# Alxaline/BraTS21

Hardware: AMD Instinct MI355X
Metric: train patches/sec (4x128^3, width-48) (higher is better)
Workload: dtype bf16; 1 GPU; equiunet width=48, batch=2/GPU of 4x128^3 synthetic patches, fwd + deep-supervision Dice + bwd + ranger (BASELINE.json configs[1]); global_batch=2, parallelism=dp1

## Files before the change

### brats21_amd/_lib.py

```python
import ctypes
import os
import re

_HERE = os.path.dirname(os.path.abspath(__file__))
LIB_PATH = os.environ.get("BRATS_HIP_LIB") or os.path.join(_HERE, "libbrats_hip.so")
HEADER_PATH = os.path.join(os.path.dirname(_HERE), "include", "brats_hip.h")

F32, BF16, F16, X3_BF16, X3_F16 = 0, 1, 2, 3, 4
ACT_NONE, ACT_RELU, ACT_LEAKY, ACT_ELU, ACT_SWISH, ACT_MISH = 0, 1, 2, 3, 4, 5
PACK_FWD, PACK_DGRAD = 0, 1


class BratsHipError(RuntimeError):
    pass


_C = {"p": ctypes.c_void_p, "i": ctypes.c_int, "f": ctypes.c_float, "d": ctypes.c_double, "z": ctypes.c_size_t}

def _parse_header():
    txt = open(HEADER_PATH).read()
    txt = re.sub(r"/\*.*?\*/", " ", txt, flags=re.S)
    sigs = {}
    for m in re.finditer(r"(const char\s*\*|size_t|int)\s+(brats_[a-z0-9_]+)\s*\(([^)]*)\)\s*;", txt):
        ret, name, args = m.group(1), m.group(2), m.group(3).strip()
        spec = ""
        if args and args != "void":
            for a in args.split(","):
                a = a.strip()
                if "*" in a or "brats_stream_t" in a:
                    spec += "p"
                elif a.startswith("size_t"):
                    spec += "z"
                elif a.startswith("double"):
                    spec += "d"
                elif a.startswith("float"):
                    spec += "f"
                elif a.startswith("int"):
                    spec += "i"
                else:
                    raise BratsHipError(f"cannot bind argument '{a}' of {name}")
        sigs[name] = ("s" if "char" in ret else ("z" if ret == "size_t" else "i"), spec)
    return sigs

# ... 51 lines not shown
```

### brats21_amd/csrc/dice.hip

```cpp
#include "common.hpp"

__global__ void dice_stats_kernel(const float* __restrict__ x, const float* __restrict__ t, float* __restrict__ part, int K,
                                  size_t voxels) {
  const int nk = blockIdx.y, k = nk % K;
  const float* xp = x + (size_t)nk * voxels;
  const float* tp = t + (size_t)nk * voxels;
  float s0 = 0.f, s1 = 0.f, s2 = 0.f;
  const size_t v4 = voxels / 4;
  for (size_t i = (size_t)blockIdx.x * blockDim.x + threadIdx.x; i < v4; i += (size_t)gridDim.x * blockDim.x) {
    const f32x4 xv = ((const f32x4*)xp)[i], tv = ((const f32x4*)tp)[i];
#pragma unroll
    for (int j = 0; j < 4; ++j) {
      const float p = 1.f / (1.f + __expf(-xv[j]));
      s0 += tv[j] * p;
      s1 += p * p;
      s2 += tv[j] * tv[j];
    }
  }
  if (blockIdx.x == 0) {
    for (size_t i = v4 * 4 + threadIdx.x; i < voxels; i += blockDim.x) {
      const float p = 1.f / (1.f + __expf(-xp[i]));
      s0 += tp[i] * p; s1 += p * p; s2 += tp[i] * tp[i];
    }
  }
// ... 68 lines not shown
  }
  if (blockIdx.x == 0) {
    for (size_t i = v4 * 4 + threadIdx.x; i < voxels; i += blockDim.x) {
      const float p = 1.f / (1.f + __expf(-xp[i]));
      dp[i] = (a * tp[i] + b2 * p) * p * (1.f - p);
    }
  }
}

constexpr int DICE_MAX_BLOCKS = 512;
extern "C" size_t brats_dice_ws_floats(int N, int K) { return (size_t)N * DICE_MAX_BLOCKS * K * 3; }

extern "C" int brats_dice_stats(const float* logits, const float* target, float* sums , float* ws, int N, int K,
                                size_t voxels, brats_stream_t s) {
  if (!logits || !target || !sums || !ws || N <= 0 || K <= 0) BRATS_FAIL(BRATS_E_ARG, "dice_stats: bad argument");
  hipStream_t st = (hipStream_t)s;
  size_t gx = (voxels / 4 + 255) / 256 / 4;
  gx = gx < 1 ? 1 : (gx > DICE_MAX_BLOCKS ? DICE_MAX_BLOCKS : gx);
  hipLaunchKernelGGL(dice_stats_kernel, dim3((unsigned)gx, N * K), dim3(256), 0, st, logits, target, ws, K, voxels);
  brats_ordered_sum(ws, sums, N * (int)gx, K * 3, st);
  BRATS_CHECK_LAUNCH();
  return 0;
}

extern "C" int brats_dice_grad(const float* logits, const float* target, const float* coef ,
                               float* dlogits, int N, int K, size_t voxels, brats_stream_t s) {
  if (!logits || !target || !coef || !dlogits) BRATS_FAIL(BRATS_E_ARG, "dice_grad: null pointer");
  size_t gx = (voxels / 4 + 255) / 256 / 4;
  gx = gx < 1 ? 1 : (gx > 2048 ? 2048 : gx);
  hipLaunchKernelGGL(dice_grad_kernel, dim3((unsigned)gx, N * K), dim3(256), 0, (hipStream_t)s, logits, target, coef, dlogits, K, voxels);
  BRATS_CHECK_LAUNCH();
  return 0;
}
```

### brats21_amd/engine.py

```python
import torch

from . import ops
from .evaluate import Evaluator
from .losses import DiceLoss, deep_supervision_loss, fused_deep_supervision_dice


class TrainStep:

    def __init__(self, model, optimizer, criterion=None, amp=True, buckets=None, fused_dice=True, jaccard=False,
                 max_grad_norm=None, amp_dtype=torch.bfloat16, scaler=None):
        self.model, self.optimizer, self.amp, self.buckets = model, optimizer, amp, buckets
        self.fused, self.jaccard, self.max_grad_norm = fused_dice and criterion is None, jaccard, max_grad_norm
        self.criterion = criterion if criterion is not None else DiceLoss(jaccard=jaccard)
        self.amp_dtype = amp_dtype
        self.scaler = scaler
        self._params = None
        if amp and amp_dtype == torch.float16 and scaler is None:
            self.scaler = torch.amp.GradScaler("cuda")

    def loss(self, outputs, target):
        if self.fused:
            return fused_deep_supervision_dice(outputs, target, jaccard=self.jaccard)
        return deep_supervision_loss(self.criterion, outputs, target)[0]

    def _zero_grad(self):
        params = self._params
        if params is None:
            params = self._params = list(self.model.parameters())
        for p in params:
            p.grad = None

    def __call__(self, image, target):
        self._zero_grad()
        with torch.autocast("cuda", dtype=self.amp_dtype, enabled=self.amp):
            outputs = self.model(image)
            loss = self.loss(outputs, target)
        if self.scaler is not None and self.amp:
            self.scaler.scale(loss).backward()
            if self.buckets is not None:
                self.buckets.finish()
            if self.max_grad_norm is not None:
                self.scaler.unscale_(self.optimizer)
                torch.nn.utils.clip_grad_norm_(self.model.parameters(), self.max_grad_norm)
            self.scaler.step(self.optimizer)
            self.scaler.update()
            return loss
        loss.backward()
        if self.buckets is not None:
            self.buckets.finish()
        if self.max_grad_norm is not None:
            torch.nn.utils.clip_grad_norm_(self.model.parameters(), self.max_grad_norm)
        self.optimizer.step()
        return loss


class GraphedTrainStep:

    def __init__(self, step, warmup=2, multi_rank_capture=None):
        if getattr(step, "scaler", None) is not None and step.amp:
            if not (getattr(step.optimizer, "_step_supports_amp_scaling", False) and getattr(step.optimizer, "capturable", False)) \
                    or step.max_grad_norm is not None:
                raise NotImplementedError("GraphedTrainStep: a TrainStep with a GradScaler (amp_dtype=torch.float16) captures only with "
                                          "an optimizer that implements the GradScaler protocol on the device "
                                          "(brats21_amd.optim.Ranger2020(capturable=True)) and without gradient clipping; otherwise use "
                                          "the eager TrainStep for fp16, or bf16 / model.precision='x3' for graph replay")
        if step.buckets is not None:
            import os
            import torch.distributed as dist
# ... 47 lines not shown
```

### brats21_amd/losses.py

```python
import torch
import torch.nn as nn


class DiceLoss(nn.Module):
    def __init__(self, jaccard=False, smooth_nr=1e-5, smooth_dr=1e-5):
        super().__init__()
        self.jaccard, self.smooth_nr, self.smooth_dr = jaccard, smooth_nr, smooth_dr

    def forward(self, logits, target):
        p = torch.sigmoid(logits.float())
        t = target.float()
        axes = (0, 2, 3, 4)
        inter = (t * p).sum(axes)
        denom = (t * t).sum(axes) + (p * p).sum(axes)
        if self.jaccard:
            denom = 2.0 * (denom - inter)
        return (1.0 - (2.0 * inter + self.smooth_nr) / (denom + self.smooth_dr)).mean()


def deep_supervision_loss(criterion, outputs, target):
    if isinstance(outputs, (tuple, list)):
        heads = [outputs[0]] + list(outputs[1])
        return torch.stack([criterion(h, target) for h in heads]).mean(), outputs[0]
    return criterion(outputs, target), outputs


class _FusedDiceFn(torch.autograd.Function):

    @staticmethod
    def forward(ctx, target, jaccard, eps, *heads):
        from . import _lib
        lib = _lib.lib()
        st = torch.cuda.current_stream().cuda_stream
        t = target.contiguous().float()
        n, k = t.shape[:2]
        vox = t[0, 0].numel()
        hs = [h.contiguous().float() for h in heads]
        sums = torch.empty((len(hs), k, 3), dtype=torch.float32, device=t.device)
        ws = torch.empty(lib.brats_dice_ws_floats(n, k), dtype=torch.float32, device=t.device)
        for i, h in enumerate(hs):
            _lib.check(lib.brats_dice_stats(h.data_ptr(), t.data_ptr(), sums[i].data_ptr(), ws.data_ptr(), n, k, vox, st), "dice_stats")
        inter, p2, t2 = sums[..., 0], sums[..., 1], sums[..., 2]
        hk = float(len(hs) * k)
        if jaccard:
            den = 2.0 * (t2 + p2 - inter)
            f = 1.0 - (2.0 * inter + eps) / (den + eps)
            dden = (2.0 * inter + eps) / (den + eps) ** 2
            coef = torch.stack([(-2.0 / (den + eps) - 2.0 * dden) / hk, 2.0 * dden / hk], -1)
        else:
            den = t2 + p2
            f = 1.0 - (2.0 * inter + eps) / (den + eps)
            coef = torch.stack([-2.0 / (den + eps) / hk, (2.0 * inter + eps) / (den + eps) ** 2 / hk], -1)
        ctx.save_for_backward(t, coef.contiguous(), *hs)
        return f.mean()

    @staticmethod
    def backward(ctx, g):
        from . import _lib
        lib = _lib.lib()
        st = torch.cuda.current_stream().cuda_stream
        t, coef, *hs = ctx.saved_tensors
        n, k = t.shape[:2]
        vox = t[0, 0].numel()
        coef = (coef * g).contiguous()
        outs = []
        for i, h in enumerate(hs):
            d = torch.empty_like(h)
            _lib.check(lib.brats_dice_grad(h.data_ptr(), t.data_ptr(), coef[i].data_ptr(), d.data_ptr(), n, k, vox, st), "dice_grad")
            outs.append(d)
        return (None, None, None) + tuple(outs)


def fused_deep_supervision_dice(outputs, target, jaccard=False, eps=1e-5):
    heads = [outputs[0]] + list(outputs[1]) if isinstance(outputs, (tuple, list)) else [outputs]
    return _FusedDiceFn.apply(target, jaccard, eps, *heads)
```

### brats21_amd/networks/equiunet.py

```python
import contextlib
import math

import os

import torch
import torch.nn as nn

from .. import ops
from .._lib import PACK_DGRAD, PACK_FWD, BratsHipError


class _ConvParams(nn.Module):

    def __init__(self, cin, cout, k, bias):
        super().__init__()
        self.weight = nn.Parameter(torch.empty(cout, cin, k, k, k))
        self.bias = nn.Parameter(torch.empty(cout)) if bias else None
        nn.init.kaiming_uniform_(self.weight, a=math.sqrt(5))
        if bias:
            bound = 1.0 / math.sqrt(cin * k * k * k)
            nn.init.uniform_(self.bias, -bound, bound)


class _NormParams(nn.Module):
# ... 415 lines not shown
        down1, p1 = cgr(m.encoder1.ConvBnRelu2, cgr(m.encoder1.ConvBnRelu1, x0, lazy=True), pool=True)
        down2, p2 = cgr(m.encoder2.ConvBnRelu2, cgr(m.encoder2.ConvBnRelu1, p1, lazy=True), pool=True)
        down3, p3 = cgr(m.encoder3.ConvBnRelu2, cgr(m.encoder3.ConvBnRelu1, p2, lazy=True), pool=True)
        down4 = cgr(m.encoder4.ConvBnRelu2, cgr(m.encoder4.ConvBnRelu1, p3, lazy=True))
        deep_heads = m.deep_supervision and not (m.skip_deep_heads_in_eval and not m.training)
        bottom = cgr(m.bottom.ConvBnRelu2, cgr(m.bottom.ConvBnRelu1, down4, lazy=True), lazy=not deep_heads)
        bottom_2 = cgr(m.bottom_2, down4, x2=bottom)
        up3 = cgr(m.decoder3.ConvBnRelu2, cgr(m.decoder3.ConvBnRelu1, down3, x2=up(bottom_2), lazy=True))
        up2 = cgr(m.decoder2.ConvBnRelu2, cgr(m.decoder2.ConvBnRelu1, down2, x2=up(up3), lazy=True))
        u1 = cgr(m.decoder1.ConvBnRelu1, down1, x2=up(up2), lazy=True)
        kact, slope_t = _unit_act(m.decoder1.ConvBnRelu2, act)
        nk = m.outconv.weight.shape[0]
        fuse_top = (m.fold_head_fwd and drop_state is None and not m.decoder1.ConvBnRelu2.batch_norm and slope_t is None and kact in ("relu", "leakyrelu") and nk <= 4
                    and (not will_bwd or (m.fold_head_bwd and ops.head_fold_ok(m.outconv.weight, kact, slope_t))))
        if fuse_top:
            y1, rec1 = _cgr_fwd(m.decoder1.ConvBnRelu2, u1, dtype, act, None, None, fp8, slots, no_act=True)
            tape.append(rec1)
            up1 = None
            outs = [ops.gn_head(y1, rec1[5], m.outconv.weight, m.outconv.bias, kact)]
        else:
            up1 = cgr(m.decoder1.ConvBnRelu2, u1)
            outs = [ops.head(up1, m.outconv.weight, m.outconv.bias, 1)]
        ctx.top_fused = fuse_top
        ctx.out_shape = tuple(outs[0].shape)
        heads = [(m.outconv, up1, 1)]
        if deep_heads:
            for hd, src, sc in ((m.deep_bottom[0], bottom, 8), (m.deep_bottom2[0], bottom_2, 8), (m.deep3[0], up3, 4),
                                (m.deep2[0], up2, 2)):
                outs.append(ops.head(src, hd.weight, hd.bias, sc))
                heads.append((hd, src, sc))
        ctx.model, ctx.dtype, ctx.tape, ctx.heads = m, dtype, tape, heads
        ctx.bufs = (down1, down2, down3, down4, bottom, bottom_2, up3, up2, up1)
        ctx.nparams = len(params)
        return tuple(outs)

    @staticmethod
    def _backward(ctx, *douts):
        m, dtype, tape = ctx.model, ctx.dtype, ctx.tape
        act, f = m.act, m.features
        names = {p: i for i, p in enumerate(m.parameters())}
        grads = {}
        down1, down2, down3, down4, bottom, bottom_2, up3, up2, up1 = ctx.bufs
        rec = {r[0]: r for r in tape}

        fp8 = m.conv_fp8 if ops.is16(dtype) else None
        slots = _AmaxSlots(32, douts[0].device) if (fp8 == "all" or ops.x3_mode() == ops.X3F) else None

        drop_state = ctx.drop_state

        def cbw(unit, dz, need_dx=True, head=None, pool=None, first=None):
            bst = rec[first] if (first is not None and m.fold_bwd_stats and drop_state is None) else None
            drop = (m.dropout_p, drop_state, m._unit_ids[unit]) if drop_state is not None else None
            return _cgr_bwd(rec[unit], dz, dtype, act, grads, names, need_dx, m._grad_sink, fp8, slots, m._grad_dest, head, pool, bst,
                            drop)

        def level_bwd(unit, down, d_pooled, d_skip, need_dx=True, first=None):
            idx = getattr(down, "_pool_argmax", None)
            kact, slope_t = _unit_act(unit, act)
            if (idx is not None and m.fold_pool_bwd and drop_state is None and not unit.batch_norm and slope_t is None
                    and kact in ("relu", "leakyrelu")):
                return cbw(unit, None, need_dx, pool=(d_skip, d_pooled, idx), first=first)
            return cbw(unit, ops.maxpool2_bwd(down, d_pooled, dx_skip=d_skip), need_dx, first=first)

        dsrc = {}
        top = None
        for (hd, src, sc), dout in zip(ctx.heads, douts):
            if dout is None and hd is m.outconv and ctx.top_fused:
                dout = torch.zeros((ctx.out_shape), dtype=torch.float32, device=douts_device(douts))
            if dout is None:
                continue
            if hd is m.outconv and (ctx.top_fused or (m.fold_head_bwd and drop_state is None and not m.decoder1.ConvBnRelu2.batch_norm
                                                       and ops.head_fold_ok(hd.weight, *_unit_act(m.decoder1.ConvBnRelu2, act)))):
                top = (hd, dout)
                continue
            dx, dw, db = ops.head_bwd(src, hd.weight, dout, sc)
            grads[names[hd.weight]] = dw
            grads[names[hd.bias]] = db
            if m._grad_sink is not None:
                m._grad_sink(names[hd.weight], dw)
                m._grad_sink(names[hd.bias], db)
            key = src.data_ptr()
            dsrc[key] = dx if key not in dsrc else dsrc[key] + dx

        def extra(t):
            return dsrc.get(t.data_ptr())

        def plus(a, b):
            return a if b is None else a + b

        def blk(b):
            return b.ConvBnRelu1, b.ConvBnRelu2

        c1, c2 = blk(m.decoder1)
        d_c1 = cbw(c2, None, head=top, first=c1) if top is not None else cbw(c2, extra(up1) if extra(up1) is not None else torch.zeros_like(up1), first=c1)
        d_skip1, d_u1 = cbw(c1, d_c1)
        d_up2 = plus(ops.upsample_bwd(d_u1, 2), extra(up2))
        c1, c2 = blk(m.decoder2)
        d_skip2, d_u2 = cbw(c1, cbw(c2, d_up2, first=c1))
# ... 113 lines not shown
```

### brats21_amd/networks/equiunet_assp.py

```python
import warnings

import os

import torch
import torch.nn as nn
import torch.nn.functional as F

from .. import ops
from .._lib import PACK_DGRAD, PACK_FWD, BratsHipError
from .equiunet import douts_device, _AmaxSlots, _ConvParams, _PackedWeightsModule, _inherit_amax


class EvoNorm3D(nn.Module):

    def __init__(self, c):
        super().__init__()
        self.gamma = nn.Parameter(torch.ones(1, c, 1, 1, 1))
        self.beta = nn.Parameter(torch.zeros(1, c, 1, 1, 1))
        self.v = nn.Parameter(torch.ones(1, c, 1, 1, 1))
        self.register_buffer("running_var", torch.ones(1, c, 1, 1, 1))


class _SEParams(nn.Module):

# ... 322 lines not shown
        br2, _, rbr2 = _conv_evo_fwd(cx, m.bridge2.conv, m.bridge2.evo, down2, out=cat2[..., :h1], uid=uid(m.bridge2))
        br3, _, rbr3 = _conv_evo_fwd(cx, m.bridge3.conv, m.bridge3.evo, down3, out=cat3[..., :h2], uid=uid(m.bridge3))
        uc3, _, ru3 = _conv_evo_fwd(cx, m.upconv3.conv, m.upconv3.evo, assp, uid=uid(m.upconv3))
        ops.upsample(uc3, 2, out=cat3[..., h2:])
        cat_amax(cat3, br3, uc3)
        up3, rd3 = _block_fwd(cx, m.decoder3, cat3)
        uc2, _, ru2 = _conv_evo_fwd(cx, m.upconv2.conv, m.upconv2.evo, up3, uid=uid(m.upconv2))
        ops.upsample(uc2, 2, out=cat2[..., h1:])
        cat_amax(cat2, br2, uc2)
        up2, rd2 = _block_fwd(cx, m.decoder2, cat2)
        uc1, _, ru1 = _conv_evo_fwd(cx, m.upconv1.conv, m.upconv1.evo, up2, uid=uid(m.upconv1))
        ops.upsample(uc1, 2, out=cat1[..., h0:])
        cat_amax(cat1, br1, uc1)
        nk = m.out_conv.weight.shape[0]
        fuse_top = m.fold_head_fwd and cx.drop is None and nk <= 4 and (not will_bwd or (m.fold_head_bwd and nk == 3))
        if fuse_top:
            logits, rd1 = _block_fwd(cx, m.decoder1, cat1, head=m.out_conv)
            up1 = None
            outs = [logits]
        else:
            up1, rd1 = _block_fwd(cx, m.decoder1, cat1)
            outs = [ops.head(up1, m.out_conv.weight, m.out_conv.bias, 1)]
        ctx.top_fused = fuse_top
        ctx.out_shape = tuple(outs[0].shape)
        heads = [(m.out_conv, up1, 1)]
        if m.deep_supervision and not (m.skip_deep_heads_in_eval and not m.training):
            for hd, src, sc in ((m.deep3[0], up3, 4), (m.deep2[0], up2, 2)):
                outs.append(ops.head(src, hd.weight, hd.bias, sc))
                heads.append((hd, src, sc))
        ctx.cx, ctx.heads, ctx.nparams = cx, heads, len(params)
        ctx.recs = dict(rb1=rb1, rb2=rb2, rb3=rb3, rb4=rb4, ra=ra, rk1=rk1, rbr1=rbr1, rbr2=rbr2, rbr3=rbr3, ru3=ru3,
                        ru2=ru2, ru1=ru1, rd3=rd3, rd2=rd2, rd1=rd1)
        ctx.bufs = (down1, down2, down3, up3, up2, up1)
        return tuple(outs)

    @staticmethod
    def _backward(ctx, *douts):
        cx, R = ctx.cx, ctx.recs
        m = cx.m
        cx.x3s = ops.x3_mode() == ops.X3F and cx.dtype == torch.float32
        f = m.features
        h0, h1, h2 = f[0] // 2, f[1] // 2, f[2] // 2
        down1, down2, down3, up3, up2, up1 = ctx.bufs
        dsrc = {}
        top = None
        for (hd, src, sc), dout in zip(ctx.heads, douts):
            if dout is None and hd is m.out_conv and ctx.top_fused:
                dout = torch.zeros((ctx.out_shape), dtype=torch.float32, device=douts_device(douts))
            if dout is None:
                continue
            if hd is m.out_conv and (ctx.top_fused or (m.fold_head_bwd and cx.drop is None and hd.weight.shape[0] == 3)):
                top = (hd, dout)
                continue
            dx, dw, db = ops.head_bwd(src, hd.weight, dout, sc)
            cx.put(hd.weight, dw)
            cx.put(hd.bias, db)
            dsrc[src.data_ptr()] = dx

        def plus(a, t):
            b = dsrc.get(t.data_ptr())
            return a if b is None else a + b

        dcat1 = _block_bwd(cx, R["rd1"], None, head=top) if top is not None else _block_bwd(cx, R["rd1"], dsrc[up1.data_ptr()] if up1.data_ptr() in dsrc else torch.zeros_like(up1))
        d_up2 = plus(_conv_evo_bwd(cx, R["ru1"], ops.upsample_bwd(dcat1[..., h0:], 2)), up2)
        dcat2 = _block_bwd(cx, R["rd2"], d_up2)
        d_up3 = plus(_conv_evo_bwd(cx, R["ru2"], ops.upsample_bwd(dcat2[..., h1:], 2)), up3)
        dcat3 = _block_bwd(cx, R["rd3"], d_up3)
        d_assp = _conv_evo_bwd(cx, R["ru3"], ops.upsample_bwd(dcat3[..., h2:], 2))
        d_acat = _conv_evo_bwd(cx, R["rk1"], d_assp)
        d_down4 = _aspp_bwd(cx, m.aspp, R["ra"], d_acat)
        def level_bwd(rec, down, d_pooled, d_skip, need_dx=True):
            idx = getattr(down, "_pool_argmax", None)
            if idx is not None and m.fold_pool_bwd and cx.drop is None:
                return _block_bwd(cx, rec, None, need_dx, pool=(d_skip, d_pooled, idx, True))
            return _block_bwd(cx, rec, ops.maxpool2_bwd(down, d_pooled, dx_skip=d_skip, with_avg=True), need_dx)

        d_p3 = _block_bwd(cx, R["rb4"], d_down4)
        d_p2 = level_bwd(R["rb3"], down3, d_p3, _conv_evo_bwd(cx, R["rbr3"], dcat3[..., :h2]))
# ... 94 lines not shown
```

### brats21_amd/ops.py

```python
import contextlib
import weakref

import numpy as np
import torch

from . import _lib
from ._lib import ACT_LEAKY, ACT_NONE, ACT_RELU, BF16, F16, F32, PACK_DGRAD, PACK_FWD, X3_BF16, X3_F16

ACTS = {"none": ACT_NONE, "relu": ACT_RELU, "leakyrelu": ACT_LEAKY, "elu": _lib.ACT_ELU, "swish": _lib.ACT_SWISH,
        "mish": _lib.ACT_MISH}


class KernelTimer:

    def __init__(self):
        self.records = {}

    def span(self, key):
        return _Span(self, key)

    def summary(self):
        torch.cuda.synchronize()
        out = {}
        for key, evs in self.records.items():
            ms = [a.elapsed_time(b) for a, b in evs]
            out[key] = (len(ms), sum(ms) / len(ms), sum(ms))
        return out


class _Span:
    def __init__(self, timer, key):
        self.timer, self.key = timer, key

# ... 771 lines not shown
        return dx
    _lib.check(_lib.lib().brats_maxpool2_bwd(ptr, p, None, 0, dptr, dp, sptr, sp, dx.data_ptr(), c, _code(x.dtype), n, c,
                                             d, h, w, int(with_avg), _stream()), "maxpool2_bwd")
    return dx


def upsample(x, scale=2, out=None):
    ptr, c, p = _desc(x)
    n, d, h, w, _ = x.shape
    if out is None:
        out = new_act(n, d * scale, h * scale, w * scale, c, x.dtype, x.device)
    optr, oc, op = _desc(out)
    _lib.check(_lib.lib().brats_upsample_fwd(ptr, p, optr, op, _code(x.dtype), n, c, d, h, w, scale, _stream()),
               "upsample_fwd")
    return out


def set_upsample_bwd_fused(mode):
    return _lib.lib().brats_upsample_bwd_set_fused(mode)


def upsample_bwd(dy, scale=2):
    dptr, c, dp = _desc(dy)
    n, do, ho, wo, _ = dy.shape
    d, h, w = do // scale, ho // scale, wo // scale
    code = _code(dy.dtype)
    ws = torch.empty(_lib.lib().brats_upsample_bwd_ws_bytes(code, n, c, d, h, w, scale), dtype=torch.uint8, device=dy.device)
    dx = new_act(n, d, h, w, c, dy.dtype, dy.device)
    _lib.check(_lib.lib().brats_upsample_bwd(dptr, dp, dx.data_ptr(), c, ws.data_ptr(), code, n, c, d, h, w, scale,
                                             _stream()), "upsample_bwd")
    return dx


def head(x, weight, bias, scale=1):
    ptr, c, p = _desc(x)
    n, d, h, w, _ = x.shape
    k = weight.shape[0]
    wf = weight.detach().reshape(k, c).contiguous().float()
    out = torch.empty((n, k, d * scale, h * scale, w * scale), dtype=torch.float32, device=x.device)
    low = torch.empty((n, k, d, h, w), dtype=torch.float32, device=x.device) if scale > 1 else None
    _lib.check(_lib.lib().brats_head_fwd(ptr, p, wf.data_ptr(), _f32(bias.detach()) if bias is not None else None,
                                         low.data_ptr() if low is not None else None, out.data_ptr(), _code(x.dtype), n, c,
                                         k, d, h, w, scale, _stream()), "head_fwd")
    return out


def gn_head(y, scale_shift, weight, bias, act="relu", slope=0.01):
    ptr, c, p = _desc(y)
    n, d, h, w, _ = y.shape
    k = weight.shape[0]
    wf = weight.detach().reshape(k, c).contiguous().float()
    out = torch.empty((n, k, d, h, w), dtype=torch.float32, device=y.device)
    _lib.check(_lib.lib().brats_gn_head_fwd(ptr, p, scale_shift.data_ptr(), ACTS[act], slope, wf.data_ptr(),
                                            _f32(bias.detach()) if bias is not None else None, out.data_ptr(), _code(y.dtype), n, c,
                                            k, d * h * w, _stream()), "gn_head_fwd")
    return out


def head_bwd(x, weight, dout, scale=1, want_dx=True):
    ptr, c, p = _desc(x)
    n, d, h, w, _ = x.shape
    k = weight.shape[0]
    wf = weight.detach().reshape(k, c).contiguous().float()
    dout = dout.contiguous().float()
    nbytes = _lib.lib().brats_head_bwd_ws_bytes(n, c, k, d, h, w, scale)
    ws = torch.empty(max(nbytes, 4) // 4, dtype=torch.float32, device=x.device)
    dx = new_act(n, d, h, w, c, x.dtype, x.device) if want_dx else None
    dw = torch.empty((k, c), dtype=torch.float32, device=x.device)
    db = torch.empty(k, dtype=torch.float32, device=x.device)
    _lib.check(_lib.lib().brats_head_bwd(ptr, p, wf.data_ptr(), dout.data_ptr(), ws.data_ptr(),
                                         dx.data_ptr() if dx is not None else None, c, dw.data_ptr(), db.data_ptr(),
# ... 304 lines not shown
```

### include/brats_hip.h

```cpp
#ifndef BRATS_HIP_H
#define BRATS_HIP_H
#include <stddef.h>
#include <stdint.h>

#ifdef __cplusplus
extern "C" {
#endif

typedef void* brats_stream_t;

enum { BRATS_F32 = 0, BRATS_BF16 = 1, BRATS_F16 = 2, BRATS_X3_BF16 = 3, BRATS_X3_F16 = 4 };
enum { BRATS_E_ARG = -1, BRATS_E_UNSUPPORTED = -2, BRATS_E_HIP = -3 };
enum { BRATS_ACT_NONE = 0, BRATS_ACT_RELU = 1, BRATS_ACT_LEAKY = 2, BRATS_ACT_ELU = 3, BRATS_ACT_SWISH = 4, BRATS_ACT_MISH = 5 };

#define BRATS_ABI_VERSION 7
int brats_abi_version(void);
const char* brats_last_error(void);

int brats_dropout(const void* x, int xpitch, void* out, int opitch, int dtype, size_t voxels, int C, float p,
                  const void* state, int unit, brats_stream_t s);

int brats_ncdhw_to_ndhwc(const float* src, void* dst, int dtype, int N, int C, int cpad, int dst_pitch,
                         int D, int H, int W, brats_stream_t s);
int brats_ndhwc_to_ncdhw(const void* src, int src_pitch, float* dst, int dtype, int N, int C,
// ... 187 lines not shown
                       int N, int C, int D, int H, int W, int scale, brats_stream_t s);
int brats_upsample_bwd_set_fused(int mode);

int brats_head_fwd(const void* x, int xpitch, const float* w , const float* b, float* lowres ,
                   float* out , int dtype, int N, int C, int K,
                   int D, int H, int W, int scale, brats_stream_t s);
int brats_gn_head_fwd(const void* y, int ypitch, const float* scale_shift, int act, float slope, const float* w ,
                      const float* b, float* out, int dtype, int N, int C, int K, int voxels, brats_stream_t s);
int brats_evonorm_head_fwd(const void* y, int ypitch, const float* scale_shift, const float* w , const float* b,
                           float* out, int dtype, int N, int C, int K, int voxels, brats_stream_t s);
size_t brats_head_bwd_ws_bytes(int N, int C, int K, int D, int H, int W, int scale);
int brats_head_bwd(const void* x, int xpitch, const float* w, const float* dout, float* ws,
                   void* dx, int dxpitch, float* dw, float* db, int dtype, int N, int C, int K,
                   int D, int H, int W, int scale, brats_stream_t s);

int brats_sw_gather(const float* src, float* dst, const int* windows, int B, int C, int D, int H, int W,
                    int rd, int rh, int rw, int pad_z, int pad_y, int pad_x, float cval, int pad_mode, brats_stream_t s);
int brats_sw_accumulate(const float* prob, const float* importance, float* out, float* count, int K,
                        int Dp, int Hp, int Wp, int rd, int rh, int rw, int n, int z0, int y0, int x0,
                        brats_stream_t s);
int brats_sw_accumulate_multi(const float* prob, const float* importance, float* out, float* count, const int* windows,
                              int B, int NB, int K, int Dp, int Hp, int Wp, int rd, int rh, int rw, brats_stream_t s);
int brats_sw_finalize(const float* out, const float* count, float* dst, int NK, int Dp, int Hp, int Wp,
                      int D, int H, int W, int pad_z, int pad_y, int pad_x, brats_stream_t s);

int brats_spatial_signed_perm(const float* src, float* dst, int planes, int s0, int s1, int s2,
                              int p0, int p1, int p2, int f0, int f1, int f2, int mode, brats_stream_t s);

size_t brats_dice_ws_floats(int N, int K);
int brats_dice_stats(const float* logits, const float* target, float* sums , float* ws, int N, int K,
                     size_t voxels, brats_stream_t s);
int brats_dice_grad(const float* logits, const float* target, const float* coef ,
                    float* dlogits, int N, int K, size_t voxels, brats_stream_t s);

int brats_pad_crop(const float* src, float* dst, int planes, int sd, int sh, int sw, int dd, int dh,
                   int dw, int oz, int oy, int ox, float fill, brats_stream_t s);
int brats_post_threshold(const float* prob, const float* img, float* seg, uint8_t* labels, int N, int K,
                         int C, size_t voxels, float scale, float thresh, brats_stream_t s);
int brats_overlap_counts(const float* pred, const float* target, unsigned long long* counts, int NK,
                         size_t voxels, brats_stream_t s);

size_t brats_cc_ws_bytes(int N, int D, int H, int W);
int brats_cc_filter(uint8_t* labels, int N, int D, int H, int W, int min_size, void* ws, brats_stream_t s);
size_t brats_rare_fill_ws_bytes(int N, int D, int H, int W);
int brats_rare_fill(uint8_t* labels, int N, int D, int H, int W, int axis, int max_count, void* ws,
                    brats_stream_t s);

size_t brats_hausdorff_ws_bytes(int NK, int D, int H, int W);
int brats_hausdorff(const float* pred, const float* target, int NK, int D, int H, int W, double percentile, int directed,
                    float* out, void* ws, brats_stream_t s);

typedef struct {
  void* param;
  const void* grad;
  void* exp_avg;
  void* exp_avg_sq;
  void* slow;
  long long numel;
  int rowlen;
  int row_base;
  float neg_step;
  float wd;
  int flags;
  int chunk_base;
} brats_ranger_tensor;
typedef struct {
// ... 41 lines not shown
```

Baseline: 144.3 patches/s.

## Fuse trilinear upsampling of deep-supervision heads into multi-head Dice kernels

Deep-supervision heads now stay at low resolution (LowResHead), and new kernels trilinearly interpolate them on the fly from LDS-staged rows. One pass computes Dice statistics for all heads at once, a single-block kernel finishes the coefficients on device, and a fused gradient kernel writes every head's dlogits. This avoids materialising full-resolution upsampled logits and cuts the per-head launches and host-side torch arithmetic. The cost is extra interpolation arithmetic, LDS staging and synchronisation per tile, and more complex gradient routing back to the low-res heads.

Result: slower. 140.0 patches/s (-3.0%).

```diff
diff --git a/brats21_amd/_lib.py b/brats21_amd/_lib.py
--- a/brats21_amd/_lib.py
+++ b/brats21_amd/_lib.py
@@ -9,6 +9,7 @@
 F32, BF16, F16, X3_BF16, X3_F16 = 0, 1, 2, 3, 4
 ACT_NONE, ACT_RELU, ACT_LEAKY, ACT_ELU, ACT_SWISH, ACT_MISH = 0, 1, 2, 3, 4, 5
 PACK_FWD, PACK_DGRAD = 0, 1
+E_ARG, E_UNSUPPORTED, E_HIP = -1, -2, -3
 
 
 class BratsHipError(RuntimeError):
diff --git a/brats21_amd/csrc/dice.hip b/brats21_amd/csrc/dice.hip
--- a/brats21_amd/csrc/dice.hip
+++ b/brats21_amd/csrc/dice.hip
@@ -124,3 +124,348 @@
   BRATS_CHECK_LAUNCH();
   return 0;
 }
+
+struct Lerp { int i0, i1; float w0, w1; };
+DEVI Lerp lerp_coef(int o, int in_len, float scale) {
+  const float src = scale * (float)o;
+  Lerp l;
+  l.i0 = (int)src;
+  if (l.i0 > in_len - 1) l.i0 = in_len - 1;
+  l.i1 = l.i0 + (l.i0 < in_len - 1 ? 1 : 0);
+  l.w1 = fminf(fmaxf(src - (float)l.i0, 0.f), 1.f);
+  l.w0 = 1.f - l.w1;
+  return l;
+}
+static inline float ac_scale(int in_len, int out_len) { return out_len > 1 ? (float)(in_len - 1) / (float)(out_len - 1) : 0.f; }
+
+constexpr int DICE_MAX_HEADS = 5;
+constexpr int DICE_KMAX = 4;
+constexpr int DICE_GRAD_ROWS = 32;
+struct DiceHead { const float* x; float* dx; int D, H, W, sc, nz, ny, rows, xc; float sd, sh, sw; };
+struct DiceHeads { DiceHead h[DICE_MAX_HEADS]; int n; };
+
+struct DiceBox { int zl0, zc, yl0, yc; };
+DEVI DiceBox dice_box(const DiceHead& h, int za, int zb, int ya, int yb) {
+  DiceBox b;
+  b.zl0 = lerp_coef(za, h.D, h.sd).i0;
+  b.zc = lerp_coef(zb, h.D, h.sd).i1 - b.zl0 + 1;
+  b.yl0 = lerp_coef(ya, h.H, h.sh).i0;
+  b.yc = lerp_coef(yb, h.H, h.sh).i1 - b.yl0 + 1;
+  if (b.zc > h.nz) b.zc = h.nz;
+  if (b.yc > h.ny) b.yc = h.ny;
+  return b;
+}
+DEVI void dice_stage_x(const DiceHead& h, float* sm) {
+  const int Wo = h.W * h.sc;
+  int* xi = (int*)(sm + h.xc);
+  float* xw0 = sm + h.xc + Wo;
+  float* xw1 = xw0 + Wo;
+  for (int x = threadIdx.x; x < Wo; x += blockDim.x) {
+    const Lerp lx = lerp_coef(x, h.W, h.sw);
+    xi[x] = lx.i0;
+    xw0[x] = lx.w0;
+    xw1[x] = lx.w1;
+  }
+}
+DEVI void dice_stage_rows(const DiceHead& h, const DiceBox& b, size_t plane, float* sm) {
+  const int Wp = h.W + 1, per = b.yc * Wp;
+  const float* low = h.x + plane * h.D * h.H * h.W;
+  for (int idx = threadIdx.x; idx < b.zc * per; idx += blockDim.x) {
+    const int pz = idx / per, rem = idx % per, r = rem / Wp, x = rem % Wp;
+    sm[h.rows + (pz * h.ny + r) * Wp + x] = low[((size_t)(b.zl0 + pz) * h.H + (b.yl0 + r)) * h.W + (x < h.W ? x : h.W - 1)];
+  }
+}
+DEVI f32x4 dice_interp(const DiceHead& h, const DiceBox& b, const float* sm, int z, int y, int x0) {
+  const int Wp = h.W + 1, Wo = h.W * h.sc;
+  const Lerp lz = lerp_coef(z, h.D, h.sd), ly = lerp_coef(y, h.H, h.sh);
+  const float wzy[4] = {lz.w0 * ly.w0, lz.w0 * ly.w1, lz.w1 * ly.w0, lz.w1 * ly.w1};
+  auto cl = [](int v, int n) { return v < 0 ? 0 : (v < n ? v : n - 1); };
+  const int p0 = cl(lz.i0 - b.zl0, b.zc) * h.ny, p1 = cl(lz.i1 - b.zl0, b.zc) * h.ny;
+  const int r0 = cl(ly.i0 - b.yl0, b.yc), r1 = cl(ly.i1 - b.yl0, b.yc);
+  const float* rows = sm + h.rows;
+  const float* rp[4] = {rows + (p0 + r0) * Wp, rows + (p0 + r1) * Wp, rows + (p1 + r0) * Wp, rows + (p1 + r1) * Wp};
+  typedef __attribute__((ext_vector_type(4))) int i32x4;
+  const i32x4 i0 = *(const i32x4*)(sm + h.xc + x0);
+  const f32x4 w0 = *(const f32x4*)(sm + h.xc + Wo + x0), w1 = *(const f32x4*)(sm + h.xc + 2 * Wo + x0);
+  f32x4 r;
+#pragma unroll
+  for (int j = 0; j < 4; ++j) {
+    float acc = 0.f;
+#pragma unroll
+    for (int k = 0; k < 8; ++k) {
+      const float wgt = wzy[k >> 1] * ((k & 1) ? w1[j] : w0[j]);
+      acc += wgt * rp[k >> 1][i0[j] + (k & 1)];
+    }
+    r[j] = acc;
+  }
+  return r;
+}
+
+__global__ void __launch_bounds__(256) dice_stats_multi_kernel(DiceHeads hs, const float* __restrict__ t, float* __restrict__ part, int K,
+                                                               int Do, int Ho, int Wo) {
+  extern __shared__ __attribute__((aligned(16))) float dsm[];
+  __shared__ float r[2 * DICE_MAX_HEADS + 1][256];
+  const int nk = blockIdx.y, k = nk % K;
+  const size_t voxels = (size_t)Do * Ho * Wo;
+  const unsigned v4 = (unsigned)(voxels / 4), W4 = Wo / 4;
+  const f32x4* tp = (const f32x4*)(t + (size_t)nk * voxels);
+#pragma unroll
+  for (int h = 0; h < DICE_MAX_HEADS; ++h)
+    if (h < hs.n && hs.h[h].sc > 1) dice_stage_x(hs.h[h], dsm);
+  float s0[DICE_MAX_HEADS], s1[DICE_MAX_HEADS], s2 = 0.f;
+#pragma unroll
+  for (int h = 0; h < DICE_MAX_HEADS; ++h) s0[h] = s1[h] = 0.f;
+  for (unsigned c = blockIdx.x; c * 256u < v4; c += gridDim.x) {
+    const unsigned f0 = c * 256u, f1 = f0 + 255u < v4 ? f0 + 255u : v4 - 1u;
+    const unsigned R0 = f0 / W4, R1 = f1 / W4;
+    const int za = R0 / Ho, zb = R1 / Ho;
+    const int ya = za == zb ? (int)(R0 % Ho) : 0, yb = za == zb ? (int)(R1 % Ho) : Ho - 1;
+    DiceBox box[DICE_MAX_HEADS];
+    __syncthreads();
+#pragma unroll
+    for (int h = 0; h < DICE_MAX_HEADS; ++h)
+      if (h < hs.n && hs.h[h].sc > 1) {
+        box[h] = dice_box(hs.h[h], za, zb, ya, yb);
+        dice_stage_rows(hs.h[h], box[h], nk, dsm);
+      }
+    __syncthreads();
+    const unsigned i = f0 + threadIdx.x;
+    if (i < v4) {
+      const unsigned R = i / W4;
+      const int x0 = (int)(i % W4) * 4, z = R / Ho, y = R % Ho;
+      const f32x4 tv = tp[i];
+#pragma unroll
+      for (int j = 0; j < 4; ++j) s2 += tv[j] * tv[j];
+#pragma unroll
+      for (int h = 0; h < DICE_MAX_HEADS; ++h)
+        if (h < hs.n) {
+          const f32x4 xv = hs.h[h].sc > 1 ? dice_interp(hs.h[h], box[h], dsm, z, y, x0)
+                                          : ((const f32x4*)(hs.h[h].x + (size_t)nk * voxels))[i];
+#pragma unroll
+          for (int j = 0; j < 4; ++j) {
+            const float p = 1.f / (1.f + __expf(-xv[j]));
+            s0[h] += tv[j] * p;
+            s1[h] += p * p;
+          }
+        }
+    }
+  }
+#pragma unroll
+  for (int h = 0; h < DICE_MAX_HEADS; ++h) { r[2 * h][threadIdx.x] = s0[h]; r[2 * h + 1][threadIdx.x] = s1[h]; }
+  r[2 * DICE_MAX_HEADS][threadIdx.x] = s2;
+  __syncthreads();
+  for (int m = 128; m > 0; m >>= 1) {
+    if ((int)threadIdx.x < m) {
+#pragma unroll
+      for (int q = 0; q < 2 * DICE_MAX_HEADS + 1; ++q) r[q][threadIdx.x] += r[q][threadIdx.x + m];
+    }
+    __syncthreads();
+  }
+  const size_t per_head = (size_t)(gridDim.y / K) * gridDim.x * K * 3;
+  if ((int)threadIdx.x < 3 * hs.n) {
+    const int h = threadIdx.x / 3, q = threadIdx.x % 3;
+    part[h * per_head + (((size_t)(nk / K) * gridDim.x + blockIdx.x) * K + k) * 3 + q] = r[q < 2 ? 2 * h + q : 2 * DICE_MAX_HEADS][0];
+  }
+}
+
+__global__ void __launch_bounds__(1024) dice_finish_kernel(const float* __restrict__ part, float* __restrict__ sums, float* __restrict__ coef,
+                                                           float* __restrict__ f, int heads, int K, int nb, int jaccard, float eps) {
+  __shared__ float sm[32][33];
+  __shared__ float tot[DICE_MAX_HEADS * DICE_KMAX * 3];
+  const int total = K * 3, entries = heads * total;
+  const int e = threadIdx.x & 31, g = threadIdx.x >> 5;
+  for (int e0 = 0; e0 < entries; e0 += 32) {
+    const int ei = e0 + e;
+    float s = 0.f;
+    if (ei < entries) {
+      const float* src = part + (size_t)(ei / total) * nb * total + ei % total;
+      int b = g;
+      for (; b + 7 * 32 < nb; b += 8 * 32) {
+        float v[8];
+#pragma unroll
+        for (int u = 0; u < 8; ++u) v[u] = src[(size_t)(b + 32 * u) * total];
+#pragma unroll
+        for (int u = 0; u < 8; ++u) s += v[u];
+      }
+      for (; b < nb; b += 32) s += src[(size_t)b * total];
+    }
+    __syncthreads();
+    sm[g][e] = s;
+    __syncthreads();
+    if (g == 0 && ei < entries) {
+#pragma unroll
+      for (int q = 1; q < 32; ++q) s += sm[q][e];
+      sums[ei] = s;
+      tot[ei] = s;
+    }
+  }
+  __syncthreads();
+  if ((int)threadIdx.x < heads * K) {
+    const float inter = tot[threadIdx.x * 3], p2 = tot[threadIdx.x * 3 + 1], t2 = tot[threadIdx.x * 3 + 2];
+    const float inv_hk = 1.f / (float)(heads * K);
+    const float num = 2.f * inter + eps;
+    float c0, c1, den;
+    if (jaccard) {
+      den = 2.f * (t2 + p2 - inter) + eps;
+      const float dden = num / (den * den);
+      c0 = ((1.f / den) * -2.f - 2.f * dden) * inv_hk;
+      c1 = (2.f * dden) * inv_hk;
+    } else {
+      den = t2 + p2 + eps;
+      c0 = ((1.f / den) * -2.f) * inv_hk;
+      c1 = (num / (den * den)) * inv_hk;
+    }
+    f[threadIdx.x] = 1.f - num / den;
+    coef[threadIdx.x * 2] = c0;
+    coef[threadIdx.x * 2 + 1] = c1;
+  }
+}
+
+__global__ void __launch_bounds__(256) dice_grad_multi_kernel(DiceHeads hs, const float* __restrict__ t, const float* __restrict__ coef,
+                                                              const float* __restrict__ gscale, int K, int Do, int Ho, int Wo) {
+  extern __shared__ __attribute__((aligned(16))) float dsm[];
+  const int nk = blockIdx.z, k = nk % K, z = blockIdx.y, y0 = blockIdx.x * DICE_GRAD_ROWS;
+  const int rows = Ho - y0 < DICE_GRAD_ROWS ? Ho - y0 : DICE_GRAD_ROWS, W4 = Wo / 4;
+  const size_t voxels = (size_t)Do * Ho * Wo, base = (size_t)nk * voxels + ((size_t)z * Ho + y0) * Wo;
+  const float g = gscale[0];
+  DiceBox box[DICE_MAX_HEADS];
+  float a[DICE_MAX_HEADS], b2[DICE_MAX_HEADS];
+#pragma unroll
+  for (int h = 0; h < DICE_MAX_HEADS; ++h)
+    if (h < hs.n) {
+      a[h] = coef[(h * K + k) * 2] * g;
+      b2[h] = 2.f * (coef[(h * K + k) * 2 + 1] * g);
+      if (hs.h[h].sc > 1) {
+        box[h] = dice_box(hs.h[h], z, z, y0, y0 + rows - 1);
+        dice_stage_x(hs.h[h], dsm);
+        dice_stage_rows(hs.h[h], box[h], nk, dsm);
+      }
+    }
+  __syncthreads();
+  for (int it = threadIdx.x; it < rows * W4; it += blockDim.x) {
+    const int yr = it / W4, x0 = (it % W4) * 4;
+    const size_t off = base + (size_t)yr * Wo + x0;
+    const f32x4 tv = *(const f32x4*)(t + off);
+#pragma unroll
+    for (int h = 0; h < DICE_MAX_HEADS; ++h)
+      if (h < hs.n) {
+        const f32x4 xv = hs.h[h].sc > 1 ? dice_interp(hs.h[h], box[h], dsm, z, y0 + yr, x0) : *(const f32x4*)(hs.h[h].x + off);
+        f32x4 o;
+#pragma unroll
+        for (int j = 0; j < 4; ++j) {
+          const float p = 1.f / (1.f + __expf(-xv[j]));
+          o[j] = (a[h] * tv[j] + b2[h] * p) * p * (1.f - p);
+        }
+        *(f32x4*)(hs.h[h].dx + off) = o;
+      }
+  }
+}
+
+static int g_dice_multi = -1;
+extern "C" int brats_dice_set_multi(int mode) {
+  const int old = g_dice_multi;
+  g_dice_multi = mode;
+  return old;
+}
+
+static unsigned dice_multi_gx(size_t voxels) {
+  size_t gx = (voxels / 4 + 255) / 256 / 4;
+  return (unsigned)(gx < 1 ? 1 : (gx > DICE_MAX_BLOCKS ? DICE_MAX_BLOCKS : gx));
+}
+struct DiceSpan { size_t rows, slices; };
+static DiceSpan dice_stats_span(int Do, int Ho, int Wo) {
+  const size_t plane = (size_t)Ho * Wo;
+  DiceSpan sp;
+  sp.rows = 1024 % Wo == 0 ? 1024 / Wo : 1024 / Wo + 2;
+  sp.slices = plane % 1024 == 0 ? 1 : (1024 % plane == 0 ? 1024 / plane : 1024 / plane + 2);
+  if (sp.slices > (size_t)Do) sp.slices = Do;
+  return sp;
+}
+static DiceSpan dice_grad_span(int Ho) { return DiceSpan{(size_t)(Ho < DICE_GRAD_ROWS ? Ho : DICE_GRAD_ROWS), 1}; }
+static size_t dice_head_lds(DiceHead& h, DiceSpan sp, size_t at) {
+  const size_t nz = sp.slices == 1 ? 2 : (sp.slices - 1) / h.sc + 4;
+  const size_t ny = sp.slices == 1 ? (sp.rows - 1) / h.sc + 4 : (size_t)h.H;
+  h.nz = (int)(nz > (size_t)h.D ? h.D : nz);
+  h.ny = (int)(ny > (size_t)h.H ? h.H : ny);
+  h.rows = (int)at;
+  h.xc = (int)(at + ((size_t)h.nz * h.ny * (h.W + 1) + 3) / 4 * 4);
+  return (size_t)h.xc + (size_t)3 * h.W * h.sc - at;
+}
+static int dice_heads(DiceHeads& hs, const float* const* heads, float* const* dlogits, const int* dims, int nheads, int K, int Do,
+                      int Ho, int Wo, DiceSpan sp, size_t static_lds, size_t* lds_bytes, const char* what) {
+  if (g_dice_multi == 0) BRATS_FAIL(BRATS_E_UNSUPPORTED, "%s: switched off (brats_dice_set_multi)", what);
+  if (nheads > DICE_MAX_HEADS || K > DICE_KMAX) BRATS_FAIL(BRATS_E_UNSUPPORTED, "%s: at most %d heads of %d classes", what, DICE_MAX_HEADS, DICE_KMAX);
+  const size_t voxels = (size_t)Do * Ho * Wo;
+  if (voxels % 4 || Wo % 4 || voxels / 4 >= (1u << 30)) BRATS_FAIL(BRATS_E_UNSUPPORTED, "%s: width and volume must be multiples of 4", what);
+  size_t at = 0;
+  hs.n = nheads;
+  for (int i = 0; i < nheads; ++i) {
+    DiceHead& h = hs.h[i];
+    h = DiceHead{heads[i], dlogits ? dlogits[i] : nullptr, dims[4 * i], dims[4 * i + 1], dims[4 * i + 2], dims[4 * i + 3], 0, 0, 0, 0, 0.f, 0.f, 0.f};
+    if (!h.x || (dlogits && !h.dx) || h.sc < 1 || h.D < 1 || h.H < 1 || h.W < 1) BRATS_FAIL(BRATS_E_ARG, "%s: bad head %d", what, i);
+    if (h.D * h.sc != Do || h.H * h.sc != Ho || h.W * h.sc != Wo) BRATS_FAIL(BRATS_E_UNSUPPORTED, "%s: head %d is not of the target's full size", what, i);
+    if (h.sc == 1) continue;
+    h.sd = ac_scale(h.D, Do); h.sh = ac_scale(h.H, Ho); h.sw = ac_scale(h.W, Wo);
+    at += dice_head_lds(h, sp, at);
+  }
+  *lds_bytes = at * sizeof(float);
+  if (*lds_bytes + static_lds > 64 * 1024) BRATS_FAIL(BRATS_E_UNSUPPORTED, "%s: heads of width %d need more than 64 KB of LDS", what, Wo);
+  return 0;
+}
+
+extern "C" int brats_dice_multi_head_ok(int K, int D, int H, int W, int scale) {
+  if (g_dice_multi == 0 || K < 1 || K > DICE_KMAX || scale < 1 || D < 1 || H < 1 || W < 1) return 0;
+  const int Do = D * scale, Ho = H * scale, Wo = W * scale;
+  const size_t voxels = (size_t)Do * Ho * Wo;
+  if (voxels % 4 || Wo % 4 || voxels / 4 >= (1u << 30) || Do > 65535) return 0;
+  DiceHead h{nullptr, nullptr, D, H, W, scale, 0, 0, 0, 0, 0.f, 0.f, 0.f};
+  const size_t a = dice_head_lds(h, dice_stats_span(Do, Ho, Wo), 0);
+  const size_t b = dice_head_lds(h, dice_grad_span(Ho), 0);
+  const size_t stat = sizeof(float) * (2 * DICE_MAX_HEADS + 1) * 256;
+  return (DICE_MAX_HEADS - 1) * a * sizeof(float) + stat <= 64 * 1024 && (DICE_MAX_HEADS - 1) * b * sizeof(float) <= 64 * 1024;
+}
+
+extern "C" size_t brats_dice_multi_ws_floats(int N, int K, int heads) { return (size_t)heads * N * DICE_MAX_BLOCKS * K * 3; }
+
+extern "C" int brats_dice_stats_multi(const float* const* heads, const int* dims , int nheads, const float* target,
+                                      float* ws, int N, int K, int Do, int Ho, int Wo, brats_stream_t s) {
+  if (!heads || !dims || !target || !ws || nheads < 1 || N <= 0 || K <= 0 || Do < 1 || Ho < 1 || Wo < 1)
+    BRATS_FAIL(BRATS_E_ARG, "dice_stats_multi: bad argument");
+  DiceHeads hs;
+  size_t lds = 0;
+  if (int rc = dice_heads(hs, heads, nullptr, dims, nheads, K, Do, Ho, Wo, dice_stats_span(Do, Ho, Wo), sizeof(float) * (2 * DICE_MAX_HEADS + 1) * 256, &lds,
+                          "dice_stats_multi"))
+    return rc;
+  if (N * K > 65535) BRATS_FAIL(BRATS_E_UNSUPPORTED, "dice_stats_multi: too many planes");
+  const unsigned gx = dice_multi_gx((size_t)Do * Ho * Wo);
+  hipLaunchKernelGGL(dice_stats_multi_kernel, dim3(gx, N * K), dim3(256), lds, (hipStream_t)s, hs, target, ws, K, Do, Ho, Wo);
+  BRATS_CHECK_LAUNCH();
+  return 0;
+}
+
+extern "C" int brats_dice_finish(const float* ws, float* sums , float* coef , float* f ,
+                                 int nheads, int N, int K, size_t voxels, int jaccard, float eps, brats_stream_t s) {
+  if (!ws || !sums || !coef || !f || nheads < 1 || nheads > DICE_MAX_HEADS || N <= 0 || K < 1 || K > DICE_KMAX)
+    BRATS_FAIL(BRATS_E_ARG, "dice_finish: bad argument");
+  hipLaunchKernelGGL(dice_finish_kernel, dim3(1), dim3(1024), 0, (hipStream_t)s, ws, sums, coef, f, nheads, K,
+                     N * (int)dice_multi_gx(voxels), jaccard, eps);
+  BRATS_CHECK_LAUNCH();
+  return 0;
+}
+
+extern "C" int brats_dice_grad_multi(const float* const* heads, const int* dims , int nheads, const float* target,
+                                     const float* coef , const float* g , float* const* dlogits,
+                                     int N, int K, int Do, int Ho, int Wo, brats_stream_t s) {
+  if (!heads || !dims || !target || !coef || !g || !dlogits || nheads < 1 || N <= 0 || K <= 0 || Do < 1 || Ho < 1 || Wo < 1)
+    BRATS_FAIL(BRATS_E_ARG, "dice_grad_multi: bad argument");
+  DiceHeads hs;
+  size_t lds = 0;
+  if (int rc = dice_heads(hs, heads, dlogits, dims, nheads, K, Do, Ho, Wo, dice_grad_span(Ho), 0,
+                          &lds, "dice_grad_multi"))
+    return rc;
+  if (Do > 65535 || N * K > 65535) BRATS_FAIL(BRATS_E_UNSUPPORTED, "dice_grad_multi: too many slices or planes");
+  hipLaunchKernelGGL(dice_grad_multi_kernel, dim3((unsigned)((Ho + DICE_GRAD_ROWS - 1) / DICE_GRAD_ROWS), (unsigned)Do, (unsigned)(N * K)),
+                     dim3(256), lds, (hipStream_t)s, hs, target, coef, g, K, Do, Ho, Wo);
+  BRATS_CHECK_LAUNCH();
+  return 0;
+}
diff --git a/brats21_amd/engine.py b/brats21_amd/engine.py
--- a/brats21_amd/engine.py
+++ b/brats21_amd/engine.py
@@ -33,7 +33,8 @@
     def __call__(self, image, target):
         self._zero_grad()
         with torch.autocast("cuda", dtype=self.amp_dtype, enabled=self.amp):
-            outputs = self.model(image)
+            with ops.lowres_deep_heads(self.fused):
+                outputs = self.model(image)
             loss = self.loss(outputs, target)
         if self.scaler is not None and self.amp:
             self.scaler.scale(loss).backward()
diff --git a/brats21_amd/losses.py b/brats21_amd/losses.py
--- a/brats21_amd/losses.py
+++ b/brats21_amd/losses.py
@@ -1,3 +1,5 @@
+import ctypes
+
 import torch
 import torch.nn as nn
 
@@ -25,33 +27,63 @@
     return criterion(outputs, target), outputs
 
 
+def _ptr_array(tensors):
+    return (ctypes.c_void_p * len(tensors))(*[x.data_ptr() for x in tensors])
+
+
+def _head_dims(srcs, scales):
+    return (ctypes.c_int * (4 * len(srcs)))(*[v for x, sc in zip(srcs, scales) for v in (*x.shape[2:], sc)])
+
+
+def _dice_terms(t, srcs, scales, jaccard, eps):
+    from . import _lib
+    lib = _lib.lib()
+    st = torch.cuda.current_stream().cuda_stream
+    n, k = t.shape[:2]
+    vox = t[0, 0].numel()
+    nh = len(srcs)
+    sums = torch.empty((nh, k, 3), dtype=torch.float32, device=t.device)
+    low = any(sc > 1 for sc in scales)
+    if t.dim() == 5 and (nh <= 5 or low):
+        ws = torch.empty(lib.brats_dice_multi_ws_floats(n, k, nh), dtype=torch.float32, device=t.device)
+        rc = lib.brats_dice_stats_multi(_ptr_array(srcs), _head_dims(srcs, scales), nh, t.data_ptr(), ws.data_ptr(), n, k,
+                                        *t.shape[2:], st)
+        if rc == 0:
+            coef = torch.empty((nh, k, 2), dtype=torch.float32, device=t.device)
+            f = torch.empty((nh, k), dtype=torch.float32, device=t.device)
+            _lib.check(lib.brats_dice_finish(ws.data_ptr(), sums.data_ptr(), coef.data_ptr(), f.data_ptr(), nh, n, k, vox,
+                                             int(bool(jaccard)), eps, st), "dice_finish")
+            return sums, coef, f, True
+        if rc != _lib.E_UNSUPPORTED or low:
+            _lib.check(rc, "dice_stats_multi")
+    ws = torch.empty(lib.brats_dice_ws_floats(n, k), dtype=torch.float32, device=t.device)
+    for i, h in enumerate(srcs):
+        _lib.check(lib.brats_dice_stats(h.data_ptr(), t.data_ptr(), sums[i].data_ptr(), ws.data_ptr(), n, k, vox, st), "dice_stats")
+    inter, p2, t2 = sums[..., 0], sums[..., 1], sums[..., 2]
+    hk = float(nh * k)
+    if jaccard:
+        den = 2.0 * (t2 + p2 - inter)
+        f = 1.0 - (2.0 * inter + eps) / (den + eps)
+        dden = (2.0 * inter + eps) / (den + eps) ** 2
+        coef = torch.stack([(-2.0 / (den + eps) - 2.0 * dden) / hk, 2.0 * dden / hk], -1)
+    else:
+        den = t2 + p2
+        f = 1.0 - (2.0 * inter + eps) / (den + eps)
+        coef = torch.stack([-2.0 / (den + eps) / hk, (2.0 * inter + eps) / (den + eps) ** 2 / hk], -1)
+    return sums, coef.contiguous(), f, False
+
+
 class _FusedDiceFn(torch.autograd.Function):
 
     @staticmethod
     def forward(ctx, target, jaccard, eps, *heads):
-        from . import _lib
-        lib = _lib.lib()
-        st = torch.cuda.current_stream().cuda_stream
+        from . import ops
         t = target.contiguous().float()
-        n, k = t.shape[:2]
-        vox = t[0, 0].numel()
-        hs = [h.contiguous().float() for h in heads]
-        sums = torch.empty((len(hs), k, 3), dtype=torch.float32, device=t.device)
-        ws = torch.empty(lib.brats_dice_ws_floats(n, k), dtype=torch.float32, device=t.device)
-        for i, h in enumerate(hs):
-            _lib.check(lib.brats_dice_stats(h.data_ptr(), t.data_ptr(), sums[i].data_ptr(), ws.data_ptr(), n, k, vox, st), "dice_stats")
-        inter, p2, t2 = sums[..., 0], sums[..., 1], sums[..., 2]
-        hk = float(len(hs) * k)
-        if jaccard:
-            den = 2.0 * (t2 + p2 - inter)
-            f = 1.0 - (2.0 * inter + eps) / (den + eps)
-            dden = (2.0 * inter + eps) / (den + eps) ** 2
-            coef = torch.stack([(-2.0 / (den + eps) - 2.0 * dden) / hk, 2.0 * dden / hk], -1)
-        else:
-            den = t2 + p2
-            f = 1.0 - (2.0 * inter + eps) / (den + eps)
-            coef = torch.stack([-2.0 / (den + eps) / hk, (2.0 * inter + eps) / (den + eps) ** 2 / hk], -1)
-        ctx.save_for_backward(t, coef.contiguous(), *hs)
+        ctx.holders = [h if isinstance(h, ops.LowResHead) else None for h in heads]
+        ctx.scales = [h.scale if isinstance(h, ops.LowResHead) else 1 for h in heads]
+        srcs = [h.low if isinstance(h, ops.LowResHead) else h.contiguous().float() for h in heads]
+        _, coef, f, ctx.multi = _dice_terms(t, srcs, ctx.scales, jaccard, eps)
+        ctx.save_for_backward(t, coef, *srcs)
         return f.mean()
 
     @staticmethod
@@ -62,6 +94,17 @@
         t, coef, *hs = ctx.saved_tensors
         n, k = t.shape[:2]
         vox = t[0, 0].numel()
+        if ctx.multi:
+            g = g.contiguous().float()
+            ds = [torch.empty_like(t) for _ in hs]
+            _lib.check(lib.brats_dice_grad_multi(_ptr_array(hs), _head_dims(hs, ctx.scales), len(hs), t.data_ptr(), coef.data_ptr(),
+                                                 g.data_ptr(), _ptr_array(ds), n, k, *t.shape[2:], st), "dice_grad_multi")
+            outs = []
+            for holder, d in zip(ctx.holders, ds):
+                if holder is not None:
+                    holder.dlogits = d
+                outs.append(None if holder is not None else d)
+            return (None, None, None) + tuple(outs)
         coef = (coef * g).contiguous()
         outs = []
         for i, h in enumerate(hs):
diff --git a/brats21_amd/networks/equiunet.py b/brats21_amd/networks/equiunet.py
--- a/brats21_amd/networks/equiunet.py
+++ b/brats21_amd/networks/equiunet.py
@@ -471,6 +471,7 @@
         ctx.model, ctx.dtype, ctx.tape, ctx.heads = m, dtype, tape, heads
         ctx.bufs = (down1, down2, down3, down4, bottom, bottom_2, up3, up2, up1)
         ctx.nparams = len(params)
+        ctx.low_heads = [o if isinstance(o, ops.LowResHead) else None for o in outs]
         return tuple(outs)
 
     @staticmethod
@@ -503,6 +504,7 @@
 
         dsrc = {}
         top = None
+        douts = tuple(lh.take_dlogits() if lh is not None else d for lh, d in zip(ctx.low_heads, douts))
         for (hd, src, sc), dout in zip(ctx.heads, douts):
             if dout is None and hd is m.outconv and ctx.top_fused:
                 dout = torch.zeros((ctx.out_shape), dtype=torch.float32, device=douts_device(douts))
diff --git a/brats21_amd/networks/equiunet_assp.py b/brats21_amd/networks/equiunet_assp.py
--- a/brats21_amd/networks/equiunet_assp.py
+++ b/brats21_amd/networks/equiunet_assp.py
@@ -378,6 +378,7 @@
         ctx.recs = dict(rb1=rb1, rb2=rb2, rb3=rb3, rb4=rb4, ra=ra, rk1=rk1, rbr1=rbr1, rbr2=rbr2, rbr3=rbr3, ru3=ru3,
                         ru2=ru2, ru1=ru1, rd3=rd3, rd2=rd2, rd1=rd1)
         ctx.bufs = (down1, down2, down3, up3, up2, up1)
+        ctx.low_heads = [o if isinstance(o, ops.LowResHead) else None for o in outs]
         return tuple(outs)
 
     @staticmethod
@@ -390,6 +391,7 @@
         down1, down2, down3, up3, up2, up1 = ctx.bufs
         dsrc = {}
         top = None
+        douts = tuple(lh.take_dlogits() if lh is not None else d for lh, d in zip(ctx.low_heads, douts))
         for (hd, src, sc), dout in zip(ctx.heads, douts):
             if dout is None and hd is m.out_conv and ctx.top_fused:
                 dout = torch.zeros((ctx.out_shape), dtype=torch.float32, device=douts_device(douts))
diff --git a/brats21_amd/ops.py b/brats21_amd/ops.py
--- a/brats21_amd/ops.py
+++ b/brats21_amd/ops.py
@@ -1,4 +1,5 @@
 import contextlib
+import threading
 import weakref
 
 import numpy as np
@@ -836,11 +837,46 @@
     return dx
 
 
+class LowResHead:
+
+    def __init__(self, low, scale):
+        self.low, self.scale, self.dlogits = low, scale, None
+
+    def take_dlogits(self):
+        d, self.dlogits = self.dlogits, None
+        return d
+
+
+_LOW_HEADS = threading.local()
+
+
+@contextlib.contextmanager
+def lowres_deep_heads(on=True):
+    old, _LOW_HEADS.on = getattr(_LOW_HEADS, "on", False), bool(on)
+    try:
+        yield
+    finally:
+        _LOW_HEADS.on = old
+
+
+def set_dice_multi(mode):
+    return _lib.lib().brats_dice_set_multi(mode)
+
+
+def dice_multi_head_ok(k, d, h, w, scale):
+    return bool(_lib.lib().brats_dice_multi_head_ok(k, d, h, w, scale))
+
+
 def head(x, weight, bias, scale=1):
     ptr, c, p = _desc(x)
     n, d, h, w, _ = x.shape
     k = weight.shape[0]
     wf = weight.detach().reshape(k, c).contiguous().float()
+    if scale > 1 and getattr(_LOW_HEADS, "on", False) and dice_multi_head_ok(k, d, h, w, scale):
+        low = torch.empty((n, k, d, h, w), dtype=torch.float32, device=x.device)
+        _lib.check(_lib.lib().brats_head_fwd(ptr, p, wf.data_ptr(), _f32(bias.detach()) if bias is not None else None, None,
+                                             low.data_ptr(), _code(x.dtype), n, c, k, d, h, w, 1, _stream()), "head_fwd")
+        return LowResHead(low, scale)
     out = torch.empty((n, k, d * scale, h * scale, w * scale), dtype=torch.float32, device=x.device)
     low = torch.empty((n, k, d, h, w), dtype=torch.float32, device=x.device) if scale > 1 else None
     _lib.check(_lib.lib().brats_head_fwd(ptr, p, wf.data_ptr(), _f32(bias.detach()) if bias is not None else None,
diff --git a/include/brats_hip.h b/include/brats_hip.h
--- a/include/brats_hip.h
+++ b/include/brats_hip.h
@@ -243,6 +243,16 @@
                      size_t voxels, brats_stream_t s);
 int brats_dice_grad(const float* logits, const float* target, const float* coef ,
                     float* dlogits, int N, int K, size_t voxels, brats_stream_t s);
+int brats_dice_set_multi(int mode);
+int brats_dice_multi_head_ok(int K, int D, int H, int W, int scale);
+size_t brats_dice_multi_ws_floats(int N, int K, int nheads);
+int brats_dice_stats_multi(const float* const* heads, const int* dims , int nheads, const float* target,
+                           float* ws, int N, int K, int Do, int Ho, int Wo, brats_stream_t s);
+int brats_dice_finish(const float* ws, float* sums, float* coef, float* f, int nheads, int N, int K, size_t voxels,
+                      int jaccard, float eps, brats_stream_t s);
+int brats_dice_grad_multi(const float* const* heads, const int* dims , int nheads, const float* target,
+                          const float* coef, const float* g, float* const* dlogits, int N, int K, int Do, int Ho, int Wo,
+                          brats_stream_t s);
 
 int brats_pad_crop(const float* src, float* dst, int planes, int sd, int sh, int sw, int dd, int dh,
                    int dw, int oz, int oy, int ox, float fill, brats_stream_t s);
```
